# hiroyasuakada/EgoRear

Measured on AMD Instinct MI355X. Metric: 4-view frames/sec (heatmap+MVFEx+3D lift), higher is better.
Workload: dtype f32 (fp16x2 split, 22-bit operands, fp32 accumulate)

## Files before the change

egorear_amd/csrc/egr_stem_x6.hip:

```cpp
#include "egr_common.h"
#include "egr_stem_pool.h"

namespace {

typedef __bf16 bf16x8 __attribute__((ext_vector_type(8)));
typedef _Float16 f16x8 __attribute__((ext_vector_type(8)));
typedef unsigned u32x4 __attribute__((ext_vector_type(4)));

constexpr int NW = 8, NT = NW * 64;
constexpr int TH = 2 * NW, TW = 32;
constexpr int PH = 2 * TH + 5;
constexpr int PW = 2 * TW + 5;
constexpr int PWS = 72;
constexpr int PATCH = 3 * PH * PWS;
constexpr int PLOADS = (PATCH + NT - 1) / NT;
constexpr int PPAIRS = (PATCH / 2 + NT - 1) / NT;
static_assert(PATCH % 2 == 0 && PWS % 2 == 0, "pixel pairs");
#ifndef STEM_PRESPLIT
#define STEM_PRESPLIT 1
#endif
#ifndef STEM_KS
#define STEM_KS 11
#endif
constexpr int KS = STEM_KS;
// ... 325 lines not shown
        __syncthreads();
        continue;
#endif
        if constexpr (POOL) {
            StemPool<NW> pool;
            pool.reduce(acc, sc, sh, half);
            if constexpr (PRE) {
                if (next < total) publish_max(buf ^ 1, pv2);
            }
            __syncthreads();
            pool.publish(s_patch[buf], wave, l31, half);
            if constexpr (PRE) {
                if (next < total) { patch_scale(buf ^ 1, psc, pinv); park2(buf ^ 1, pv2, psc); }
            } else {
                if (next < total) park(buf ^ 1, pv);
            }
            __syncthreads();
            pool.finish(s_patch[buf], wave, l31, half, y, n, oy0, ox0, a.ho >> 1, a.wo >> 1);
            amx = fmaxf(amx, pool.amx);
        } else {
#pragma unroll
            for (int i = 0; i < 2; ++i) {
                const int oy = oy0 + 2 * wave + i;
#pragma unroll
                for (int r = 0; r < 16; ++r) {
                    const int ox = ox0 + (r & 3) + 8 * (r >> 2) + 4 * half;
                    f32x2 v;
                    v[0] = acc[i][0][r] * sc[0] + sh[0];
                    v[1] = acc[i][1][r] * sc[1] + sh[1];
                    if (!raw) {
                        v[0] = v[0] > 0.f ? v[0] : 0.f;
                        v[1] = v[1] > 0.f ? v[1] : 0.f;
                    }
                    *reinterpret_cast<f32x2*>(&y[(((int64_t)n * a.ho + oy) * a.wo + ox) * 64 + 2 * l31]) = v;
                }
            }
            if constexpr (PRE) {
                if (next < total) publish_max(buf ^ 1, pv2);
                __syncthreads();
                if (next < total) { patch_scale(buf ^ 1, psc, pinv); park2(buf ^ 1, pv2, psc); }
            } else {
                if (next < total) park(buf ^ 1, pv);
            }
            __syncthreads();
        }
    }
    if (POOL && a.amax_out) {
        amx = wave_max(amx);
        if (lane == 0 && amx > 0.f)
            __hip_atomic_fetch_max(a.amax_out + ((blockIdx.x * NW + wave) & 63), __float_as_uint(amx), __ATOMIC_RELAXED, __HIP_MEMORY_SCOPE_AGENT);
    }
}

__global__ __launch_bounds__(64) void pack_stem_w6_kernel(const float* __restrict__ w, uint8_t* __restrict__ img) {
    const int lane = threadIdx.x, j = blockIdx.x & 1, s = blockIdx.x >> 1, grp = blockIdx.y;
    const int co = 2 * (lane & 31) + j, p = 2 * s + (lane >> 5);
    const float* wr = w + ((int64_t)grp * 64 + co) * 148;
    u32x4 h, m, l;
#pragma unroll
    for (int e = 0; e < 4; ++e) {
        float v[2];
#pragma unroll
        for (int z = 0; z < 2; ++z) {
            const int kw = 2 * e + z;
            v[z] = (p <= 20 && kw < 7) ? wr[p * 7 + kw] : 0.f;
        }
        h[e] = cvt_pk_bf16(v[0], v[1]);
        const float r0 = v[0] - bf16_lo_f32(h[e]), r1 = v[1] - bf16_hi_f32(h[e]);
        m[e] = cvt_pk_bf16(r0, r1);
        l[e] = cvt_pk_bf16(r0 - bf16_lo_f32(m[e]), r1 - bf16_hi_f32(m[e]));
    }
    uint8_t* dst = img + (int64_t)grp * WBYTES + ((s * 2 + j) * 3) * 1024 + lane * 16;
    *reinterpret_cast<u32x4*>(dst) = h;
    *reinterpret_cast<u32x4*>(dst + 1024) = m;
    *reinterpret_cast<u32x4*>(dst + 2048) = l;
}

__global__ __launch_bounds__(64) void pack_stem_wh2_kernel(const float* __restrict__ w, uint8_t* __restrict__ img, float* __restrict__ descale) {
    const int lane = threadIdx.x, j = blockIdx.x & 1, s = blockIdx.x >> 1, grp = blockIdx.y;
    const int co = 2 * (lane & 31) + j, p = 2 * s + (lane >> 5);
    const float* wr = w + ((int64_t)grp * 64 + co) * 148;
    float m = 0.f;
    for (int k = 0; k < 147; ++k) m = fmaxf(m, fabsf(wr[k]));
    float sc, inv;
    pow2_prescale(__float_as_uint(m), sc, inv);
    if (s == 0 && lane < 32) descale[grp * 64 + co] = inv;
    u32x4 h, l;
#pragma unroll
    for (int e = 0; e < 4; ++e) {
        float v[2];
#pragma unroll
        for (int z = 0; z < 2; ++z) {
            const int kw = 2 * e + z;
            v[z] = (p <= 20 && kw < 7) ? wr[p * 7 + kw] : 0.f;
        }
        unsigned hh, ll;
        split2_f16(v[0], v[1], sc, hh, ll);
        h[e] = hh;
        l[e] = ll;
    }
    uint8_t* dst = img + (int64_t)grp * WBYTES2 + ((s * 2 + j) * 2) * 1024 + lane * 16;
    *reinterpret_cast<u32x4*>(dst) = h;
    *reinterpret_cast<u32x4*>(dst + 1024) = l;
}

}

extern "C" int64_t egr_stem_wh2_bytes(void) { return WBYTES2; }

extern "C" int egr_pack_stem_wh2_f32(const float* w, int32_t groups, void* img, float* descale, void* stream) {
    if (!w || !img || !descale) return EGR_ENULL;
    if (groups <= 0 || groups > 65535 || ((uintptr_t)img & 15)) return EGR_EINVAL;
    hipLaunchKernelGGL(pack_stem_wh2_kernel, dim3(KS * 2, (unsigned)groups), dim3(64), 0, (hipStream_t)stream, w, (uint8_t*)img, descale);
    return egr_launch_status();
}

extern "C" int64_t egr_stem_w6_bytes(void) { return WBYTES; }

extern "C" int egr_pack_stem_w6_f32(const float* w, int32_t groups, void* img, void* stream) {
    if (!w || !img) return EGR_ENULL;
    if (groups <= 0 || groups > 65535 || ((uintptr_t)img & 15)) return EGR_EINVAL;
    hipLaunchKernelGGL(pack_stem_w6_kernel, dim3(KS * 2, (unsigned)groups), dim3(64), 0, (hipStream_t)stream, w, (uint8_t*)img);
    return egr_launch_status();
}

static int stem_x6_run(const float* x, egr_nmap xmap, int32_t n, int32_t h, int32_t w, const void* w6, const float* scale, const float* shift,
                       float* y, int32_t pool, int32_t groups, int64_t gx, uint32_t* amax_out, void* stream, const float* wds = nullptr);

extern "C" int egr_stem_conv7x7_h2_f32(const float* x, egr_nmap xmap, int32_t n, int32_t h, int32_t w, const void* wh2, const float* w_descale,
                                       const float* scale, const float* shift, float* y, int32_t pool, int32_t groups, int64_t gx,
                                       uint32_t* amax_out, void* stream) {
    if (!w_descale) return EGR_ENULL;
    if (amax_out && !pool) return EGR_EINVAL;
    return stem_x6_run(x, xmap, n, h, w, wh2, scale, shift, y, pool, groups, gx, amax_out, stream, w_descale);
}

extern "C" int egr_stem_conv7x7_x6_f32(const float* x, egr_nmap xmap, int32_t n, int32_t h, int32_t w, const void* w6,
                                       const float* scale, const float* shift, float* y, int32_t pool, int32_t groups, int64_t gx,
                                       void* stream) {
    return stem_x6_run(x, xmap, n, h, w, w6, scale, shift, y, pool, groups, gx, nullptr, stream);
}

extern "C" int egr_stem_conv7x7_x6_ex_f32(const float* x, egr_nmap xmap, int32_t n, int32_t h, int32_t w, const void* w6,
                                          const float* scale, const float* shift, float* y, int32_t pool, int32_t groups, int64_t gx,
                                          uint32_t* amax_out, void* stream) {
    if (amax_out && !pool) return EGR_EINVAL;
    return stem_x6_run(x, xmap, n, h, w, w6, scale, shift, y, pool, groups, gx, amax_out, stream);
}

static int stem_x6_run(const float* x, egr_nmap xmap, int32_t n, int32_t h, int32_t w, const void* w6, const float* scale, const float* shift,
                       float* y, int32_t pool, int32_t groups, int64_t gx, uint32_t* amax_out, void* stream, const float* wds) {
    if (!x || !w6 || !y || ((scale == nullptr) != (shift == nullptr))) return EGR_ENULL;
    if (pool && !scale) return EGR_EINVAL;
    if (groups <= 0 || groups > 65535 || ((uintptr_t)w6 & 15)) return EGR_EINVAL;
    if (n <= 0 || h <= 0 || w <= 0 || h % (2 * TH) != 0 || w % (2 * TW) != 0 || xmap.n_inner <= 0) return EGR_EINVAL;
    StemX6Args a;
    a.x = x; a.xmap = xmap; a.n = n; a.h = h; a.w = w; a.ho = h / 2; a.wo = w / 2;
    a.w6 = (const uint8_t*)w6; a.scale = scale; a.shift = shift; a.y = y;
    a.tiles_x = a.wo / TW; a.tiles_y = a.ho / TH;
    a.gx = gx;
    a.amax_out = amax_out;
    a.wds = wds;
    const int64_t tiles = (int64_t)n * a.tiles_x * a.tiles_y;
    if (tiles >= (1LL << 31)) return EGR_EINVAL;
    int64_t blocks = 256 / groups;
    if (blocks < 1) blocks = 1;
    if (blocks > tiles) blocks = tiles;
    hipStream_t s = (hipStream_t)stream;
    if (pool) {
        stem_pool_init<NW>(y, (int64_t)groups * n, a.ho / 2, a.wo / 2, s);
        if (wds) hipLaunchKernelGGL((stem_x6_kernel<true, 2>), dim3((unsigned)blocks, (unsigned)groups), dim3(NT), 0, s, a);
        else hipLaunchKernelGGL((stem_x6_kernel<true, 3>), dim3((unsigned)blocks, (unsigned)groups), dim3(NT), 0, s, a);
    } else {
        if (wds) hipLaunchKernelGGL((stem_x6_kernel<false, 2>), dim3((unsigned)blocks, (unsigned)groups), dim3(NT), 0, s, a);
        else hipLaunchKernelGGL((stem_x6_kernel<false, 3>), dim3((unsigned)blocks, (unsigned)groups), dim3(NT), 0, s, a);
    }
    return egr_launch_status();
}
```

egorear_amd/hip.py:

```python
from __future__ import annotations

import ctypes as C
import math
import os
import threading
from typing import Optional, Union

import torch

_HERE = os.path.dirname(os.path.abspath(__file__))
LIB_PATH = os.environ.get("EGR_LIB") or os.path.join(_HERE, "csrc", "libegorear_hip.so")

ACT_NONE, ACT_RELU, ACT_GELU = 0, 1, 2
RES_NONE, RES_BEFORE_ACT, RES_AFTER_ACT, RES_UP2_BEFORE_ACT = 0, 1, 2, 3



import contextlib
import dataclasses
import sys
import types


class _on_default:
# ... 58 lines not shown
        return self.replace(w_format="f16", h2=True, layer_h2=True)

    @_on_default
    def fast_training(self) -> "LaunchPolicy":
        return self.fast().replace(train_one_product=True)

    @property
    def fp16_scheme(self) -> bool:
        return self.w_format in ("f16x2", "f16")


POLICY = LaunchPolicy.from_env()
_POLICY_TLS = threading.local()


def policy() -> LaunchPolicy:
    cur = getattr(_POLICY_TLS, "cur", None)
    return cur if cur is not None else POLICY


@contextlib.contextmanager
def use_policy(p: Optional[LaunchPolicy]):
    if p is None:
        yield
        return
    old = getattr(_POLICY_TLS, "cur", None)
    _POLICY_TLS.cur = p
    try:
        yield
    finally:
        _POLICY_TLS.cur = old


def install_policy_properties(module_name: str, mapping: dict) -> None:
    def make(field):
        return property(lambda self: getattr(policy(), field), lambda self, v: setattr(POLICY, field, v))
    mod = sys.modules[module_name]
    mod.__class__ = type("_PolicyModule", (types.ModuleType,), {name: make(field) for name, field in mapping.items()})


install_policy_properties(__name__, {
    "H2": "h2", "X6_MIN_ROWS": "x6_min_rows", "X6_MIN_FLOPS": "x6_min_flops", "X6_TRAIN_MIN_ROWS": "x6_train_min_rows",
    "X6_TRAIN_MIN_FLOPS": "x6_train_min_flops", "CHAIN": "chain", "CHAIN_MIN_ROWS": "chain_min_rows", "CHAIN_BIG": "chain_big",
    "CHAIN_BIG_MIN_ROWS": "chain_big_min_rows", "WGRAD_X6": "wgrad_x6", "WGRAD_FORCE": "wgrad_force"})

EXPORTS = [
    "egr_conv2d_nhwc_f32", "egr_stem_conv7x7_f32", "egr_maxpool_nhwc_f32", "egr_upsample2x_nhwc_f32",
    "egr_avgpool_nhwc_f32", "egr_argmax_rows_f32", "egr_layernorm_f32", "egr_joint_mha_f32", "egr_msda_gather_f32",
    "egr_fisheye_project_f32", "egr_linear_smallk_f32", "egr_jqa_sum_f32", "egr_tokens_to_nhwc_f32", "egr_version",
    "egr_device_arch", "egr_conv_force_config", "egr_preprocess_u8_f32", "egr_pose_metrics_f32", "egr_gt_heatmap_f32", "egr_conv_debug_stamps", "egr_conv2d_wgrad_f32", "egr_conv2d_masked_f32", "egr_up2_relu_head_f32",
    "egr_msda_fwd_f32", "egr_msda_bwd_f32", "egr_w6_elems", "egr_pack_w6_f32", "egr_pack_w6_many_f32", "egr_joint_layer_f32",
    "egr_preprocess_fused_u8_f32", "egr_preprocess_band_rows", "egr_preprocess_last_kernel", "egr_conv_set_persist", "egr_stem_conv7x7_pool_f32",
    "egr_stem_w6_bytes", "egr_pack_stem_w6_f32", "egr_stem_conv7x7_x6_f32", "egr_wgrad_last_kernel", "egr_conv_last_kernel", "egr_conv_set_tap", "egr_conv_set_tapx", "egr_conv_set_splitk_fused", "egr_fisheye_project2_f32", "egr_pack_layer_w_f32", "egr_pack_layer_wh2_f32",
    "egr_conv2d_nhwc_ex_f32", "egr_wh2_elems", "egr_pack_wh2_f32", "egr_absmax_f32", "egr_stem_conv7x7_x6_ex_f32", "egr_stem_wh2_bytes", "egr_pack_stem_wh2_f32", "egr_stem_conv7x7_h2_f32",
    "egr_pack_wh2_many_f32", "egr_conv2d_masked_ex_f32", "egr_conv2d_wgrad_ex_f32", "egr_wgrad_last_h2", "egr_wgrad_last_planes",
    "egr_wstream_image_bytes", "egr_pack_wstream_f32", "egr_linear_wstream_workspace_bytes", "egr_linear_wstream_f32", "egr_conv1x1_chain_f32",
    "egr_jqa_query_f32", "egr_pose_query_f32", "egr_layer_set_planes", "egr_head_set_persist", "egr_heatmap_metrics_f32",
    "egr_conv_plan", "egr_soft_argmax_f32", "egr_soft_argmax_bwd_f32", "egr_coord_l1_f32",
    "egr_triangulate_f32", "egr_triangulate_bwd_f32", "egr_volume_fuse_f32", "egr_volume_fuse_bwd_f32",
    "egr_peaks_f32", "egr_consensus_f32", "egr_skeleton_fit_f32", "egr_bone_lengths_f32", "egr_skeleton_resize_f32",
    "egr_trajectory_smooth_f32", "egr_trajectory_smooth_bwd_f32", "egr_rig_refine_f32", "egr_rig_refine_workspace_bytes",
    "egr_ray_track_f32", "egr_ray_track_workspace_bytes",
]


class NMap(C.Structure):
    _fields_ = [("n_inner", C.c_int32), ("stride_inner", C.c_int64), ("stride_outer", C.c_int64)]


class ConvDesc(C.Structure):
    _fields_ = [
        ("n", C.c_int32), ("h", C.c_int32), ("w", C.c_int32), ("cin", C.c_int32), ("cout", C.c_int32),
        ("kh", C.c_int32), ("kw", C.c_int32), ("stride", C.c_int32), ("pad", C.c_int32),
        ("ho", C.c_int32), ("wo", C.c_int32), ("ldx", C.c_int32), ("ldy", C.c_int32), ("ldr", C.c_int32),
        ("xmap", NMap), ("ymap", NMap), ("rmap", NMap),
        ("act", C.c_int32), ("res_mode", C.c_int32), ("out_nchw", C.c_int32), ("split_k", C.c_int32),
        ("groups", C.c_int32),
        ("gx", C.c_int64), ("gw", C.c_int64), ("gp", C.c_int64), ("gy", C.c_int64), ("gr", C.c_int64),
        ("grs", C.c_int64), ("grm", C.c_int64),
        ("transposed", C.c_int32), ("w_format", C.c_int32),
    ]


class ConvAux(C.Structure):
    _fields_ = [("w_descale", C.c_void_p), ("amax_in", C.c_void_p), ("amax_out", C.c_void_p),
                ("bn_partials", C.c_void_p), ("bn_tiles_out", C.c_void_p), ("bn_capacity", C.c_int64),
                ("in_mode", C.c_int32), ("in_up2_out", C.c_void_p)]


IN_PLAIN, IN_UP2_RELU = 0, 1


class ConvPlan(C.Structure):
    _fields_ = [(n, C.c_int32) for n in ("route", "bm", "bn", "variant", "planes", "tiles_m", "tiles_n", "grid_x", "grid_y", "grid_z", "block",
                                         "split_k", "ktiles_per_split", "persistent", "cls_mode", "fused_reduce", "reduce_pass", "bn_slabs")]


ROUTE_F32_TILED, ROUTE_SPLIT_TILED, ROUTE_TAP, ROUTE_TAP2, ROUTE_STREAM_1X1, ROUTE_SMALL_F32, ROUTE_TAPX = range(7)
PRE_ROUTE_LDS, PRE_ROUTE_DWORD, PRE_ROUTE_GENERIC, PRE_ROUTE_FUSED = range(4)
W_F16X2, W_F16X1, W_F16X1T = 4, 8, 16


class ChainAux(C.Structure):
    _fields_ = [("w2", C.c_void_p), ("w2_descale", C.c_void_p), ("shift1", C.c_void_p), ("cmid", C.c_int32), ("act1", C.c_int32),
                ("gw2", C.c_int64), ("gp1", C.c_int64)]


# ... 7 lines not shown
                                           "x_out", "w_ol", "b_ol", "ol_out")] +
                [("ol_n", C.c_int32), ("w_packed", C.c_int32)] +
                [(n, C.c_void_p) for n in ("lnp_g", "lnp_b", "xn_out", "w_r0", "b_r0", "w_r2", "b_r2", "anchors3d", "pred_out",
                                           "w_h0", "b_h0", "h0_out", "amax_h0")] +
                [("h0_n", C.c_int32)])


class JqaQueryDesc(C.Structure):
    _fields_ = ([(n, C.c_int32) for n in ("B", "J", "C", "groups", "kb", "pool_hw", "ol_n", "w_packed")] +
                [(n, C.c_void_p) for n in ("t", "s32", "w_hp2", "b_hp2", "w_bfb", "b_bfb", "embed", "w_q", "b_q", "w_ol", "b_ol",
                                           "x_out", "ol_out")])


class PoseQueryDesc(C.Structure):
    _fields_ = ([(n, C.c_int32) for n in ("B", "J", "C", "ol_n", "w_packed")] +
                [(n, C.c_void_p) for n in ("h1", "w_m2", "b_m2", "ctm", "cams", "w_qg0", "b_qg0", "w_qg2", "b_qg2", "w_qg4", "b_qg4",
                                           "w_ol", "b_ol", "pred_out", "anchors3d_out", "anchors2d_out", "valid_out", "x_out", "ol_out")])


def _load() -> C.CDLL:
    if not os.path.exists(LIB_PATH):
        raise ImportError(
            f"{LIB_PATH} not found: build it with `python -m egorear_amd.csrc.build` "
            "(or __graft_entry__.build()).  egorear_amd has no CPU / PyTorch fallback.")
    lib = C.CDLL(LIB_PATH)
    vp, i32, i64, f32 = C.c_void_p, C.c_int32, C.c_int64, C.c_float
    lib.egr_conv2d_nhwc_f32.argtypes = [C.POINTER(ConvDesc), vp, vp, vp, vp, vp, vp, vp, vp, vp, C.c_size_t, vp]
    lib.egr_conv2d_nhwc_ex_f32.argtypes = [C.POINTER(ConvDesc), vp, vp, vp, vp, vp, vp, vp, vp, vp, C.c_size_t, C.POINTER(ConvAux), vp]
    lib.egr_conv_plan.argtypes = [C.POINTER(ConvDesc), vp, vp, vp, vp, vp, vp, vp, vp, vp, vp, C.c_size_t, C.POINTER(ConvAux), C.POINTER(ConvPlan)]
    lib.egr_conv1x1_chain_f32.argtypes = [C.POINTER(ConvDesc), vp, vp, vp, vp, vp, C.POINTER(ConvAux), C.POINTER(ChainAux), vp]
    lib.egr_fill_f32.argtypes = [vp, f32, i64, vp]
    lib.egr_fill_f32.restype = C.c_int
    lib.egr_absmax_f32.argtypes = [vp, i64, vp, vp]
    lib.egr_wh2_elems.restype = C.c_int64
    lib.egr_wh2_elems.argtypes = [i32, i32]
    lib.egr_pack_wh2_f32.argtypes = [vp, i32, i32, i32, vp, vp, vp]
    lib.egr_stem_conv7x7_f32.argtypes = [vp, NMap, i32, i32, i32, vp, vp, vp, vp, i32, i64, vp]
    lib.egr_stem_conv7x7_pool_f32.argtypes = [vp, NMap, i32, i32, i32, vp, vp, vp, vp, i32, i64, vp]
    lib.egr_wgrad_last_kernel.argtypes = []
    lib.egr_wgrad_last_planes.argtypes = []
    lib.egr_conv_last_kernel.argtypes = []
    lib.egr_conv_set_tap.argtypes = [i32]
    lib.egr_conv_set_tapx.argtypes = [i32, i32, i32]
    lib.egr_conv_set_splitk_fused.argtypes = [i32]
    lib.egr_stem_w6_bytes.restype = C.c_int64
    lib.egr_stem_w6_bytes.argtypes = []
    lib.egr_pack_stem_w6_f32.argtypes = [vp, i32, vp, vp]
    lib.egr_stem_conv7x7_x6_f32.argtypes = [vp, NMap, i32, i32, i32, vp, vp, vp, vp, i32, i32, i64, vp]
    lib.egr_stem_conv7x7_x6_ex_f32.argtypes = [vp, NMap, i32, i32, i32, vp, vp, vp, vp, i32, i32, i64, vp, vp]
    lib.egr_stem_wh2_bytes.restype = C.c_int64
    lib.egr_stem_wh2_bytes.argtypes = []
    lib.egr_pack_stem_wh2_f32.argtypes = [vp, i32, vp, vp, vp]
    lib.egr_stem_conv7x7_h2_f32.argtypes = [vp, NMap, i32, i32, i32, vp, vp, vp, vp, vp, i32, i32, i64, vp, vp]
    lib.egr_wstream_image_bytes.restype = C.c_int64
    lib.egr_wstream_image_bytes.argtypes = [i32, i32]
    lib.egr_pack_wstream_f32.argtypes = [vp, i32, i32, vp, vp, vp]
    lib.egr_linear_wstream_workspace_bytes.restype = C.c_int64
    lib.egr_linear_wstream_workspace_bytes.argtypes = [i32, i32, i32]
    lib.egr_linear_wstream_f32.argtypes = [vp, i64, i32, i32, vp, vp, vp, i32, i32, vp, vp, i64, vp, vp, i64, vp]
    lib.egr_maxpool_nhwc_f32.argtypes = [vp, vp, i32, i32, i32, i32, i32, i32, i32, vp]
    lib.egr_upsample2x_nhwc_f32.argtypes = [vp, i32, vp, i32, i32, i32, i32, i32, i32, vp]
    lib.egr_avgpool_nhwc_f32.argtypes = [vp, vp, i32, i32, i32, vp]
    lib.egr_argmax_rows_f32.argtypes = [vp, i32, i32, i32, f32, vp, vp, vp, vp, vp]
    lib.egr_soft_argmax_f32.argtypes = [vp, i32, i32, i32, f32, i32, i32, f32, vp, vp, vp, vp, vp, vp, vp]
    lib.egr_soft_argmax_bwd_f32.argtypes = [vp, vp, vp, vp, vp, vp, i32, i32, i32, f32, i32, i32, i32, vp, vp]
    lib.egr_triangulate_f32.argtypes = [vp, vp, vp, vp, i32, i32, i32, f32, f32, f32, f32, vp, vp, vp, vp, vp]
    lib.egr_triangulate_bwd_f32.argtypes = [vp, vp, vp, vp, i32, i32, i32, f32, f32, f32, f32, vp, vp, vp, vp, vp]
    lib.egr_volume_fuse_f32.argtypes = [vp, vp, vp, vp, vp, vp, i32, i32, i32, i32, i32, i32, f32, f32, f32, vp, vp, vp, vp, vp, vp]
    lib.egr_volume_fuse_bwd_f32.argtypes = [vp, vp, vp, vp, vp, vp, i32, i32, i32, i32, i32, i32, f32, f32, f32, vp, vp, vp, vp]
    lib.egr_peaks_f32.argtypes = [vp, i32, i32, i32, i32, i32, i32, f32, f32, vp, vp, vp, vp, vp]
    lib.egr_consensus_f32.argtypes = [vp, vp, vp, vp, vp, i32, i32, i32, i32, f32, f32, f32, i32, f32, vp, vp, vp, vp, vp, vp, vp]
    lib.egr_skeleton_fit_f32.argtypes = [vp, vp, vp, vp, vp, vp, i32, vp, vp, i32, i32, i32, f32, f32, f32, f32, f32, f32, i32, vp, vp, vp, vp,
                                         vp, vp, vp, vp, vp]
    lib.egr_bone_lengths_f32.argtypes = [vp, vp, vp, i32, i32, vp, vp, vp, vp]
    lib.egr_skeleton_resize_f32.argtypes = [vp, vp, vp, vp, i32, i32, i32, vp, vp]
    lib.egr_trajectory_smooth_f32.argtypes = [vp, vp, vp, i32, i32, i32, f32, f32, f32, i32, i32, vp, vp, vp, vp, vp, vp, vp]
    lib.egr_trajectory_smooth_bwd_f32.argtypes = [vp, vp, vp, vp, i32, i32, i32, f32, f32, vp, vp, vp, vp]
    lib.egr_rig_refine_workspace_bytes.restype = C.c_int64
    lib.egr_rig_refine_workspace_bytes.argtypes = [i32, i32, i32]
    lib.egr_rig_refine_f32.argtypes = [vp, vp, vp, vp, i32, i32, i32, i32, f32, f32, f32, f32, i32, f32, i32, vp, i64, vp, vp, vp, vp, vp, vp,
                                       vp, vp, vp, vp]
    lib.egr_ray_track_workspace_bytes.restype = C.c_int64
    lib.egr_ray_track_workspace_bytes.argtypes = [i32, i32, i32, i32]
    lib.egr_ray_track_f32.argtypes = [vp, vp, vp, vp, i32, i32, i32, i32, f32, f32, f32, f32, f32, f32, i32, i32, C.c_double, vp, i64, vp, vp, vp,
                                      vp, vp, vp, vp]
    lib.egr_coord_l1_f32.argtypes = [vp, vp, vp, i32, i32, f32, vp, vp, vp]
    lib.egr_layernorm_f32.argtypes = [vp, vp, vp, vp, vp, i32, i32, f32, i32, vp]
    lib.egr_joint_mha_f32.argtypes = [vp, vp, i32, i32, i32, i32, f32, vp]
    lib.egr_msda_gather_f32.argtypes = [vp, i32, vp, i32, vp, vp, vp, i32, i32, i32, i32, i32, i32, vp, vp, vp, vp, i32, vp]
    lib.egr_fisheye_project_f32.argtypes = [vp, vp, vp, i32, i32, vp, vp, vp, vp]
    lib.egr_fisheye_project2_f32.argtypes = [vp, vp, vp, vp, i32, i32, vp, vp, vp, vp]
    lib.egr_linear_smallk_f32.argtypes = [vp, i64, i64, vp, vp, vp, i32, i32, i32, i32, i32, vp]
    lib.egr_jqa_sum_f32.argtypes = [vp, vp, vp, vp, i32, i32, i32, i32, vp]
    lib.egr_tokens_to_nhwc_f32.argtypes = [vp, vp, i32, i32, i32, vp]
    lib.egr_version.restype = C.c_char_p
    lib.egr_w6_elems.restype = C.c_int64
    lib.egr_device_arch.argtypes = [C.c_char_p, i32]
    lib.egr_conv_force_config.argtypes = [i32]
    lib.egr_conv_set_persist.argtypes = [i32, i32]
    lib.egr_up2_relu_head_f32.argtypes = [vp, i32, i32, i32, i32, vp, vp, i32, vp, i32, i64, i64, i32, i64, vp]
    lib.egr_conv2d_masked_f32.argtypes = [C.POINTER(ConvDesc), vp, vp, vp, vp, vp, vp, C.c_size_t, vp]
    lib.egr_conv2d_masked_ex_f32.argtypes = [C.POINTER(ConvDesc), vp, vp, vp, vp, vp, vp, C.c_size_t, C.POINTER(ConvAux), vp]
    lib.egr_conv2d_wgrad_f32.argtypes = [C.POINTER(ConvDesc), vp, vp, vp, vp, vp, C.c_size_t, i32, vp]
    lib.egr_conv2d_wgrad_ex_f32.argtypes = [C.POINTER(ConvDesc), vp, vp, vp, vp, vp, C.c_size_t, i32, vp, vp, vp]
    lib.egr_gt_heatmap_f32.argtypes = [vp, i32, C.c_double, i32, i32, vp, vp, vp]
    lib.egr_pose_metrics_f32.argtypes = [vp, vp, i32, i32, f32, i32, vp, vp, vp]
# ... 665 lines not shown
def pack_stem_w6(wpack: torch.Tensor) -> torch.Tensor:
    if wpack.dim() != 3 or wpack.shape[1:] != (64, 148) or wpack.dtype != torch.float32:
        raise RuntimeError("egorear_amd.pack_stem_w6: (groups, 64, 148) fp32 expected")
    img = torch.empty((wpack.shape[0], int(lib.egr_stem_w6_bytes())), device=wpack.device, dtype=torch.uint8)
    _launch("egr_pack_stem_w6_f32", lib.egr_pack_stem_w6_f32, _p(_cont(wpack, "stem weight")), wpack.shape[0], _p(img, torch.uint8), _stream())
    return img


def pack_wstream(w: torch.Tensor):
    if w.dim() != 2 or w.dtype != torch.float32 or w.shape[0] % 64 or w.shape[1] % 256:
        raise RuntimeError("egorear_amd.pack_wstream: (n % 64 == 0, k % 256 == 0) fp32 expected")
    n, k = w.shape
    img = torch.empty((int(lib.egr_wstream_image_bytes(n, k)),), device=w.device, dtype=torch.uint8)
    ds = torch.empty((n,), device=w.device, dtype=torch.float32)
    _launch("egr_pack_wstream_f32", lib.egr_pack_wstream_f32, _p(_cont(w, "weight")), n, k, _p(img, torch.uint8), _p(ds), _stream())
    return img, ds


def linear_wstream(x: torch.Tensor, img: torch.Tensor, descale: torch.Tensor, bias: Optional[torch.Tensor], act: int, workspace: torch.Tensor,
                   amax_out: Optional[torch.Tensor] = None) -> torch.Tensor:
    rec = getattr(x, "_egr_amax", None)
    if rec is None:
        raise RuntimeError("egorear_amd.linear_wstream: the rows carry no abs-max record")
    n = descale.numel()
    rows, k = x.shape
    if x.dtype != torch.float32 or x.stride(1) != 1 or img.numel() != 4 * n * k:
        raise RuntimeError("egorear_amd.linear_wstream: operands do not match")
    y = torch.empty((rows, n), device=x.device, dtype=torch.float32)
    for r0 in range(0, rows, 64):
        r = min(64, rows - r0)
        need = int(lib.egr_linear_wstream_workspace_bytes(r, n, k))
        if need < 0 or workspace.numel() * workspace.element_size() < need:
            raise RuntimeError(f"egorear_amd.linear_wstream: workspace of {need} bytes needed")
        xr, yr = x[r0:r0 + r], y[r0:r0 + r]
        _launch("egr_linear_wstream_f32", lib.egr_linear_wstream_f32, _p(xr), xr.stride(0), r, k, _p(img, torch.uint8), _p(descale),
                _p(bias), n, act, _p(rec, torch.int32), _p(yr), yr.stride(0), _p(amax_out, torch.int32), _p(workspace, workspace.dtype),
                workspace.numel() * workspace.element_size(), _stream(), flops=2.0 * r * n * k, nbytes=4.0 * n * k + 4.0 * r * (n + k),
                tag="h2 wstream")
    if amax_out is not None:
        y._egr_amax = amax_out
    return y


def pack_stem_wh2(wpack: torch.Tensor):
    if wpack.dim() != 3 or wpack.shape[1:] != (64, 148) or wpack.dtype != torch.float32:
        raise RuntimeError("egorear_amd.pack_stem_wh2: (groups, 64, 148) fp32 expected")
    img = torch.empty((wpack.shape[0], int(lib.egr_stem_wh2_bytes())), device=wpack.device, dtype=torch.uint8)
    ds = torch.empty((wpack.shape[0], 64), device=wpack.device, dtype=torch.float32)
    _launch("egr_pack_stem_wh2_f32", lib.egr_pack_stem_wh2_f32, _p(_cont(wpack, "stem weight")), wpack.shape[0], _p(img, torch.uint8), _p(ds), _stream())
    return img, ds


def stem_x6(img: torch.Tensor, view0: int, nviews: int, w6: torch.Tensor, scale, shift, groups: int = 1, pool: bool = False,
            amax_out: Optional[torch.Tensor] = None, w_descale: Optional[torch.Tensor] = None) -> Img:
    B, V, Cc, H, W = img.shape
    if Cc != 3:
        raise RuntimeError("egorear_amd.stem_x6: 3-channel input expected")
    _cont(img, "input image batch")
    raw = scale is None and shift is None
    if pool and raw:
        raise RuntimeError("egorear_amd.stem_x6: the fused max-pool needs the eval-mode BatchNorm scale / shift")
    h2 = w_descale is not None
    if (view0 + groups * nviews > V or w6.dtype != torch.uint8
            or w6.numel() != groups * int(lib.egr_stem_wh2_bytes() if h2 else lib.egr_stem_w6_bytes())
            or (h2 and w_descale.numel() != groups * 64)
            or (not raw and (scale.numel() != groups * 64 or shift.numel() != groups * 64))):
        raise RuntimeError("egorear_amd.stem_x6: views / weights mismatch")
    n = nviews * B
    d = 4 if pool else 2
    y = torch.empty((groups * n, H // d, W // d, 64), device=img.device, dtype=torch.float32)
    base = img.reshape(-1)[view0 * 3 * H * W:]
    xmap = NMap(B, V * 3 * H * W, 3 * H * W)
    if amax_out is not None and (not pool or amax_out.numel() != 64 or amax_out.dtype != torch.int32):
        raise RuntimeError("egorear_amd.stem_x6: the abs-max record (64 int32 slots) goes with pool=True")
    if h2:
        _launch("egr_stem_conv7x7_x6_f32", lib.egr_stem_conv7x7_h2_f32, _p(base), xmap, n, H, W, _p(_cont(w6, "stem weight"), torch.uint8),
                _p(_cont(w_descale, "stem descale")), _p(scale), _p(shift), _p(y), 1 if pool else 0, groups, nviews * 3 * H * W,
                _p(amax_out, torch.int32), _stream(),
                flops=2.0 * groups * n * (H // 2) * (W // 2) * 64 * 147, nbytes=4.0 * groups * n * (3 * H * W + (H // d) * (W // d) * 64),
                tag="h2 pool" if pool else "h2")
    else:
        _launch("egr_stem_conv7x7_x6_f32", lib.egr_stem_conv7x7_x6_ex_f32, _p(base), xmap, n, H, W, _p(_cont(w6, "stem weight"), torch.uint8), _p(scale),
                _p(shift), _p(y), 1 if pool else 0, groups, nviews * 3 * H * W, _p(amax_out, torch.int32), _stream(),
                flops=2.0 * groups * n * (H // 2) * (W // 2) * 64 * 147, nbytes=4.0 * groups * n * (3 * H * W + (H // d) * (W // d) * 64),
                tag="x6 pool" if pool else "x6")
    out = Img(y)
    out.tag(amax_out)
    return out


def maxpool(x: Img, k: int, stride: int, pad: int) -> Img:
    if not x.t.is_contiguous():
        raise RuntimeError("egorear_amd.maxpool: contiguous NHWC input expected")
    ho = (x.h + 2 * pad - k) // stride + 1
    wo = (x.w + 2 * pad - k) // stride + 1
    y = torch.empty((x.n, ho, wo, x.c), device=x.t.device, dtype=torch.float32)
    _launch("egr_maxpool_nhwc_f32", lib.egr_maxpool_nhwc_f32, _p(x.t), _p(y), x.n, x.h, x.w, x.c, k, stride, pad, _stream(),
            nbytes=4.0 * x.n * x.c * (x.h * x.w + ho * wo))
    out = Img(y)
    out.tag(x.amax)
    return out


def upsample2x(x: Img, out: Optional[Img] = None, relu: bool = False) -> Img:
    if x.n > 1 and x.nstride != x.h * x.w * x.ld:
        raise RuntimeError("egorear_amd.upsample2x: images must be densely stacked")
    if out is None:
        out = Img(torch.empty((x.n, 2 * x.h, 2 * x.w, x.c), device=x.t.device, dtype=torch.float32))
    if (out.n, out.h, out.w, out.c) != (x.n, 2 * x.h, 2 * x.w, x.c) or (out.n > 1 and out.nstride != out.h * out.w * out.ld):
        raise RuntimeError("egorear_amd.upsample2x: bad output view")
    _launch("egr_upsample2x_nhwc_f32", lib.egr_upsample2x_nhwc_f32, _p(x.t), x.ld, _p(out.t), out.ld, x.n, x.h, x.w, x.c, 1 if relu else 0, _stream(),
            nbytes=4.0 * 5 * x.n * x.h * x.w * x.c)
    out.tag(x.amax)
    return out


def up2_relu_head(lo: Img, wgt: torch.Tensor, bias: Optional[torch.Tensor], planes: torch.Tensor, ymap: NMap, gy: int, groups: int = 1):
    if not lo.t.is_contiguous() or lo.n % groups:
        raise RuntimeError("egorear_amd.up2_relu_head: dense NHWC input with groups | n expected")
    cout, cin = wgt.shape[-2], wgt.shape[-1]
    npg = lo.n // groups
    if cin != lo.c or wgt.numel() != groups * cout * cin or (bias is not None and bias.numel() != groups * cout):
        raise RuntimeError("egorear_amd.up2_relu_head: weight / bias shape")
    ho, wo = 2 * lo.h, 2 * lo.w
    last = (groups - 1) * gy + (npg - 1) // ymap.n_inner * ymap.stride_outer + min(npg - 1, ymap.n_inner - 1) * ymap.stride_inner + cout * ho * wo
    if not planes.is_contiguous() or last > planes.numel():
        raise RuntimeError("egorear_amd.up2_relu_head: output map runs outside the tensor")
    _launch("egr_up2_relu_head_f32", lib.egr_up2_relu_head_f32, _p(lo.t), lo.n, lo.h, lo.w, cin, _p(_cont(wgt, "weight")), _p(bias), cout,
            _p(planes), ymap.n_inner, ymap.stride_inner, ymap.stride_outer, groups, gy, _stream(),
# ... 930 lines not shown
```

include/egorear_hip.h:

```cpp
#ifndef EGOREAR_HIP_H
#define EGOREAR_HIP_H

#include <stddef.h>
#include <stdint.h>

#ifdef __cplusplus
extern "C" {
#endif

#define EGR_EINVAL (-1)
#define EGR_ENULL (-2)
#define EGR_EWORKSPACE (-3)

enum { EGR_ACT_NONE = 0, EGR_ACT_RELU = 1, EGR_ACT_GELU = 2 };
enum { EGR_RES_NONE = 0, EGR_RES_BEFORE_ACT = 1, EGR_RES_AFTER_ACT = 2,
       EGR_RES_UP2_BEFORE_ACT = 3  };

typedef struct {
    int32_t n_inner;
    int64_t stride_inner;
    int64_t stride_outer;
} egr_nmap;

typedef struct {
// ... 104 lines not shown
                  const float* workspace, size_t workspace_floats, const egr_conv_aux* aux, egr_conv_plan_t* out);

int egr_conv2d_wgrad_f32(const egr_conv_desc* d, const float* x, const float* dy, float* dw, float* db,
                         float* workspace, size_t workspace_floats, int32_t accumulate, void* stream);
int egr_conv2d_wgrad_ex_f32(const egr_conv_desc* d, const float* x, const float* dy, float* dw, float* db, float* workspace,
                            size_t workspace_floats, int32_t accumulate, const uint32_t* amax_x, const uint32_t* amax_dy, void* stream);
int egr_wgrad_last_h2(void);
int egr_wgrad_last_planes(void);
int egr_wgrad_last_kernel(void);

int egr_conv_force_config(int cfg);
int egr_conv_last_kernel(void);
int egr_conv_set_splitk_fused(int on);
int egr_conv_set_tap(int on);
int egr_conv_set_tapx(int32_t on, int32_t min_tiles, int32_t blocks);
int egr_conv_set_persist(int slots, int max_ktiles);

int egr_up2_relu_head_f32(const float* lo, int32_t n, int32_t h, int32_t w, int32_t cin, const float* wgt, const float* bias,
                          int32_t cout, float* planes, int32_t n_inner, int64_t stride_inner, int64_t stride_outer,
                          int32_t groups, int64_t gy, void* stream);
int egr_head_set_persist(int on);

int egr_conv_debug_stamps(unsigned long long* buf);

int egr_stem_conv7x7_f32(const float* x, egr_nmap xmap, int32_t n, int32_t h, int32_t w,
                         const float* wpack, const float* scale, const float* shift, float* y,
                         int32_t groups ,
                         int64_t gx, void* stream);

int egr_stem_conv7x7_pool_f32(const float* x, egr_nmap xmap, int32_t n, int32_t h, int32_t w,
                              const float* wpack, const float* scale, const float* shift, float* y,
                              int32_t groups, int64_t gx, void* stream);

int64_t egr_stem_w6_bytes(void);
int egr_pack_stem_w6_f32(const float* w, int32_t groups, void* w6, void* stream);
int egr_stem_conv7x7_x6_f32(const float* x, egr_nmap xmap, int32_t n, int32_t h, int32_t w,
                            const void* w6, const float* scale, const float* shift, float* y,
                            int32_t pool, int32_t groups, int64_t gx, void* stream);
int egr_stem_conv7x7_x6_ex_f32(const float* x, egr_nmap xmap, int32_t n, int32_t h, int32_t w,
                            const void* w6, const float* scale, const float* shift, float* y,
                            int32_t pool, int32_t groups, int64_t gx, uint32_t* amax_out, void* stream);
int64_t egr_wstream_image_bytes(int32_t n, int32_t k);
int egr_pack_wstream_f32(const float* w, int32_t n, int32_t k, void* img, float* descale, void* stream);
int64_t egr_linear_wstream_workspace_bytes(int32_t rows, int32_t n, int32_t k);
int egr_linear_wstream_f32(const float* x, int64_t ldx, int32_t rows, int32_t k, const void* wimg, const float* w_descale, const float* bias,
                           int32_t n, int32_t act, const uint32_t* amax_in, float* y, int64_t ldy, uint32_t* amax_out, void* workspace,
                           int64_t workspace_bytes, void* stream);

int64_t egr_stem_wh2_bytes(void);
int egr_pack_stem_wh2_f32(const float* w, int32_t groups, void* img, float* descale, void* stream);
int egr_stem_conv7x7_h2_f32(const float* x, egr_nmap xmap, int32_t n, int32_t h, int32_t w, const void* wh2, const float* w_descale,
                            const float* scale, const float* shift, float* y, int32_t pool, int32_t groups, int64_t gx,
                            uint32_t* amax_out, void* stream);

int egr_maxpool_nhwc_f32(const float* x, float* y, int32_t n, int32_t h, int32_t w, int32_t c,
                         int32_t k, int32_t stride, int32_t pad, void* stream);

int egr_upsample2x_nhwc_f32(const float* x, int32_t ldx, float* y, int32_t ldy,
                            int32_t n, int32_t h, int32_t w, int32_t c, int32_t relu, void* stream);

int egr_absmax_f32(const float* x, int64_t n, uint32_t* record, void* stream);

int egr_avgpool_nhwc_f32(const float* x, float* y, int32_t n, int32_t hw, int32_t c, void* stream);

int egr_argmax_rows_f32(const float* hm, int32_t rows, int32_t hgt, int32_t wid, float thr,
                        float* anchors , float* maxvals, uint8_t* valid, int32_t* index, void* stream);

int egr_soft_argmax_f32(const float* hm, int32_t rows, int32_t hgt, int32_t wid, float beta, int32_t mode, int32_t normalize, float thr,
                        float* coords , float* maxvals, int32_t* index, uint8_t* valid, float* stat ,
                        float* probs , void* stream);
int egr_soft_argmax_bwd_f32(const float* hm, const float* stat, const float* coords, const int32_t* index, const float* g_coords,
                            const float* g_maxvals , int32_t rows, int32_t hgt, int32_t wid, float beta, int32_t mode,
                            int32_t normalize, int32_t accumulate, float* g_hm, void* stream);
int egr_coord_l1_f32(const float* coords, const int32_t* index, const uint8_t* valid, int32_t rows, int32_t wid, float weight,
                     double* loss, float* g_coords , void* stream);

int egr_triangulate_f32(const float* coords, const float* conf, const float* cams, const float* ctm , int32_t B, int32_t V,
                        int32_t J, float sx, float sy, float threshold, float min_det_ratio, float* pts ,
                        float* cost , float* resid , uint8_t* ok , void* stream);
int egr_triangulate_bwd_f32(const float* coords, const float* conf, const float* cams, const float* ctm , int32_t B,
                            int32_t V, int32_t J, float sx, float sy, float threshold, float min_det_ratio,
                            const float* g_pts , const float* g_cost , float* g_coords, float* g_conf,
                            void* stream);

int egr_volume_fuse_f32(const float* hm, const float* conf, const float* centers, const float* cams, const float* ctm ,
                        const uint8_t* center_ok , int32_t B, int32_t V, int32_t J, int32_t H, int32_t W, int32_t G,
                        float cube, float beta, float threshold, float* pose , float* peak ,
                        int32_t* index , float* spread , uint8_t* ok , void* stream);
int egr_volume_fuse_bwd_f32(const float* hm, const float* conf, const float* centers, const float* cams, const float* ctm ,
                            const uint8_t* center_ok , int32_t B, int32_t V, int32_t J, int32_t H, int32_t W, int32_t G,
                            float cube, float beta, float threshold, const float* g_pose ,
                            const float* g_peak , float* g_hm, void* stream);

int egr_peaks_f32(const float* hm, int32_t rows, int32_t hgt, int32_t wid, int32_t K, int32_t nms_radius, int32_t refine_radius, float beta,
                  float min_score, float* coords , float* score , int32_t* index ,
                  int32_t* count , void* stream);
int egr_consensus_f32(const float* cand, const float* cscore, const int32_t* cindex, const float* cams, const float* ctm ,
                      int32_t B, int32_t V, int32_t J, int32_t K, float sx, float sy, float max_reproj, int32_t min_views,
                      float min_det_ratio, int32_t* choice , float* sel_coords ,
                      float* sel_conf , float* score , int32_t* inliers , int32_t* hyp ,
                      void* stream);

int egr_skeleton_fit_f32(const float* coords, const float* conf, const float* cams, const float* ctm ,
                         const int32_t* parents , const float* bone_length, int32_t bone_length_per_frame, const float* init,
                         const uint8_t* init_ok, int32_t B, int32_t V, int32_t J, float sx, float sy, float threshold, float min_det_ratio,
                         float lambda, float rho, int32_t iterations, float* pose , float* ray_cost ,
// ... 147 lines not shown
```

Baseline: 6973.

## Add warp-specialized stem conv kernel splitting MFMA and load/store waves

```diff
diff --git a/egorear_amd/csrc/egr_stem_x6.hip b/egorear_amd/csrc/egr_stem_x6.hip
--- a/egorear_amd/csrc/egr_stem_x6.hip
+++ b/egorear_amd/csrc/egr_stem_x6.hip
@@ -401,6 +401,292 @@
     }
 }
 
+namespace rs {
+constexpr int MW = 4;
+constexpr int LT = MW * 64;
+constexpr int LPAIRS = (PATCH / 2 + LT - 1) / LT;
+constexpr int ROWF = 16 * 64;
+constexpr int O_MAIN = 0;
+constexpr int O_NEXT = O_MAIN + 8 * ROWF * 4;
+constexpr int O_EA = O_NEXT + MW * ROWF * 4;
+constexpr int O_EB = O_EA + 8 * 64 * 4;
+constexpr int O_PMAX = O_EB + MW * 64 * 4;
+constexpr int O_PATCH = O_PMAX + 4 * MW * 4;
+constexpr int PBYTES = PATCH * 4;
+constexpr int O_W = O_PATCH + 2 * PBYTES;
+constexpr int LDS_BYTES = O_W + WBYTES2;
+static_assert(O_PATCH % 16 == 0 && O_W % 16 == 0 && LDS_BYTES <= 160 * 1024, "LDS map");
+}
+
+__global__ __launch_bounds__(NT, 1) void stem_h2_pool_rs_kernel(const StemX6Args a) {
+    using namespace rs;
+    __shared__ __attribute__((aligned(16))) uint8_t lds[LDS_BYTES];
+    const int tid = threadIdx.x, lane = tid & 63, wave = __builtin_amdgcn_readfirstlane(tid >> 6);
+    const int grp = blockIdx.y;
+    const int tpi = a.tiles_x * a.tiles_y;
+    const int total = a.n * tpi;
+    const int ntiles = (total - (int)blockIdx.x + (int)gridDim.x - 1) / (int)gridDim.x;
+    const int pho = a.ho >> 1, pwo = a.wo >> 1;
+    const auto barrier = [] { asm volatile("s_waitcnt lgkmcnt(0)\n\ts_barrier" ::: "memory"); };
+    unsigned* const s_pmax = reinterpret_cast<unsigned*>(lds + O_PMAX);
+    auto patch_scale = [&](int slot, float& s, float& inv) {
+        unsigned m = s_pmax[slot * MW + (lane & (MW - 1))];
+#pragma unroll
+        for (int o = MW / 2; o > 0; o >>= 1) {
+            const unsigned other = (unsigned)__shfl_xor((int)m, o, 64);
+            m = other > m ? other : m;
+        }
+        pow2_prescale(__builtin_amdgcn_readfirstlane(m), s, inv);
+    };
+    {
+        const u32x4* src = reinterpret_cast<const u32x4*>(a.w6 + (int64_t)grp * WBYTES2);
+        for (int i = tid; i < WBYTES2 / 16; i += NT) reinterpret_cast<u32x4*>(lds + O_W)[i] = src[i];
+    }
+
+    if (wave < MW) {
+        const int l31 = lane & 31, half = lane >> 5;
+        float sc[2], sh[2], wds[2];
+#pragma unroll
+        for (int j = 0; j < 2; ++j) {
+            sc[j] = a.scale[grp * 64 + 2 * l31 + j];
+            sh[j] = a.shift[grp * 64 + 2 * l31 + j];
+            wds[j] = a.wds[grp * 64 + 2 * l31 + j];
+        }
+        const int abase = ((2 * (4 * wave)) * PWS + 2 * l31) >> 1;
+        unsigned bbase = O_W + lane * 16;
+        asm volatile("" : "+v"(bbase));
+        float amx = 0.f;
+        barrier();
+        barrier();
+        for (int it = 0; it < ntiles; ++it) {
+            const unsigned* const ph = reinterpret_cast<const unsigned*>(lds + O_PATCH + (it & 1) * PBYTES);
+            float psc, pinv;
+            patch_scale(it & 3, psc, pinv);
+            f32x16 acc[2][2][2];
+#pragma unroll
+            for (int p = 0; p < 2; ++p)
+#pragma unroll
+                for (int i = 0; i < 2; ++i)
+#pragma unroll
+                    for (int j = 0; j < 2; ++j)
+#pragma unroll
+                        for (int r = 0; r < 16; ++r) acc[p][i][j][r] = 0.f;
+            u32x4 al[4], ah[2][4];
+            u32x4 bl[2], bh[2][2];
+            auto read_a = [&](int s, int pl, u32x4 (&d)[4]) {
+                const unsigned* const q = ph + abase + pl * (PATCH / 2) + ((half ? pair_off_t<PH>(2 * s + 1) : pair_off_t<PH>(2 * s)) >> 1);
+#pragma unroll
+                for (int i = 0; i < 4; ++i)
+#pragma unroll
+                    for (int e = 0; e < 4; ++e) d[i][e] = q[i * PWS + e];
+            };
+            auto read_b = [&](int s, int pl, u32x4 (&d)[2]) {
+#pragma unroll
+                for (int j = 0; j < 2; ++j) d[j] = *reinterpret_cast<const u32x4*>(lds + bbase + ((s * 2 + j) * 2 + pl) * 1024);
+            };
+            auto mul = [&](const u32x4 (&fa)[4], const u32x4 (&fb)[2]) {
+#pragma unroll
+                for (int i = 0; i < 4; ++i)
+#pragma unroll
+                    for (int j = 0; j < 2; ++j)
+                        acc[i >> 1][i & 1][j] = __builtin_amdgcn_mfma_f32_32x32x16_f16(__builtin_bit_cast(f16x8, fa[i]), __builtin_bit_cast(f16x8, fb[j]),
+                                                                                      acc[i >> 1][i & 1][j], 0, 0, 0);
+            };
+            read_a(0, 1, al);
+            read_b(0, 0, bh[0]);
+            read_a(0, 0, ah[0]);
+            read_b(0, 1, bl);
+#pragma unroll
+            for (int s = 0; s < KS; ++s) {
+                const int par = s & 1;
+                if (s + 1 < KS) {
+                    read_b(s + 1, 0, bh[par ^ 1]);
+                    read_a(s + 1, 0, ah[par ^ 1]);
+                }
+                __builtin_amdgcn_sched_barrier(0);
+                mul(al, bh[par]);
+                __builtin_amdgcn_sched_barrier(0);
+                if (s + 1 < KS) read_a(s + 1, 1, al);
+                __builtin_amdgcn_sched_barrier(0);
+                mul(ah[par], bl);
+                __builtin_amdgcn_sched_barrier(0);
+                if (s + 1 < KS) read_b(s + 1, 1, bl);
+                __builtin_amdgcn_sched_barrier(0);
+                mul(ah[par], bh[par]);
+                __builtin_amdgcn_sched_barrier(0);
+            }
+#pragma unroll
+            for (int p = 0; p < 2; ++p)
+#pragma unroll
+                for (int i = 0; i < 2; ++i)
+#pragma unroll
+                    for (int j = 0; j < 2; ++j) {
+                        const float dsc = pinv * wds[j];
+#pragma unroll
+                        for (int r = 0; r < 16; ++r) acc[p][i][j][r] *= dsc;
+                    }
+            StemPool<NW> pa, pb;
+            pa.reduce(acc[0], sc, sh, half);
+            pb.reduce(acc[1], sc, sh, half);
+            amx = fmaxf(amx, fmaxf(pa.amx, pb.amx));
+            barrier();
+            float* const st = reinterpret_cast<float*>(lds);
+#pragma unroll
+            for (int q = 0; q < 8; ++q) {
+                const int o = StemPool<NW>::pc(q, half) * 64 + 2 * l31;
+                f32x2 mid;
+                mid[0] = fmaxf(pb.P0[q][0], pa.P1[q][0]);
+                mid[1] = fmaxf(pb.P0[q][1], pa.P1[q][1]);
+                *reinterpret_cast<f32x2*>(&st[O_MAIN / 4 + (2 * wave) * ROWF + o]) = pa.P0[q];
+                *reinterpret_cast<f32x2*>(&st[O_MAIN / 4 + (2 * wave + 1) * ROWF + o]) = mid;
+                *reinterpret_cast<f32x2*>(&st[O_NEXT / 4 + wave * ROWF + o]) = pb.P1[q];
+            }
+            if (half) {
+                f32x2 mid;
+                mid[0] = fmaxf(pb.e0[0], pa.e1[0]);
+                mid[1] = fmaxf(pb.e0[1], pa.e1[1]);
+                *reinterpret_cast<f32x2*>(&st[O_EA / 4 + (2 * wave) * 64 + 2 * l31]) = pa.e0;
+                *reinterpret_cast<f32x2*>(&st[O_EA / 4 + (2 * wave + 1) * 64 + 2 * l31]) = mid;
+                *reinterpret_cast<f32x2*>(&st[O_EB / 4 + wave * 64 + 2 * l31]) = pb.e1;
+            }
+            barrier();
+        }
+        if (a.amax_out) {
+            amx = wave_max(amx);
+            if (lane == 0 && amx > 0.f)
+                __hip_atomic_fetch_max(a.amax_out + ((blockIdx.x * NW + wave) & 63), __float_as_uint(amx), __ATOMIC_RELAXED, __HIP_MEMORY_SCOPE_AGENT);
+        }
+    } else {
+        const int lw = wave - MW, ltid = tid - LT;
+        const float* const xg = a.x + grp * a.gx;
+        float* const y = a.y + (int64_t)grp * a.n * pho * pwo * 64;
+        int q_geo[LPAIRS], q_off[LPAIRS];
+#pragma unroll
+        for (int u = 0; u < LPAIRS; ++u) {
+            const int i = 2 * (ltid + LT * u);
+            const int ci = i / (PH * PWS);
+            const int r = i - ci * PH * PWS;
+            const int py = r / PWS, px = r - py * PWS;
+            q_geo[u] = (i < PATCH) ? ((py << 8) | px) : (1 << 30);
+            q_off[u] = (ci * a.h + py) * a.w + px;
+        }
+        auto tile_of = [&](int it) { return (int)blockIdx.x + it * (int)gridDim.x; };
+        auto fetch = [&](int tile, float (&v)[2 * LPAIRS]) {
+            const int n = tile / tpi;
+            const int t = tile - n * tpi;
+            const int ty = t / a.tiles_x, tx = t - ty * a.tiles_x;
+            const int iy0 = 2 * ty * TH - 3, ix0 = 2 * tx * TW - 3;
+            const uint64_t ip = (uint64_t)(xg + egr_map(a.xmap, n));
+            const uint32_t ip_lo = __builtin_amdgcn_readfirstlane((uint32_t)ip), ip_hi = __builtin_amdgcn_readfirstlane((uint32_t)(ip >> 32));
+            const __amdgpu_buffer_rsrc_t rx = __builtin_amdgcn_make_buffer_rsrc((void*)(((uint64_t)ip_hi << 32) | ip_lo), 0, 0x80000000u, 0x00020000);
+            const int toff = iy0 * a.w + ix0;
+            const unsigned xlim = (unsigned)(a.w < ix0 + PW ? a.w : ix0 + PW);
+#pragma unroll
+            for (int u = 0; u < LPAIRS; ++u) {
+                const int g = q_geo[u];
+                const int iy = iy0 + (g >> 8), ix = ix0 + (g & 255);
+                const bool rowok = (unsigned)iy < (unsigned)a.h;
+                const int o = (int)((unsigned)(toff + q_off[u]) * 4u);
+                const int o0 = (rowok && (unsigned)ix < xlim) ? o : (int)0x80000000;
+                const int o1 = (rowok && (unsigned)(ix + 1) < xlim) ? o + 4 : (int)0x80000000;
+                v[2 * u] = __builtin_bit_cast(float, __builtin_amdgcn_raw_buffer_load_b32(rx, o0, 0, 0));
+                v[2 * u + 1] = __builtin_bit_cast(float, __builtin_amdgcn_raw_buffer_load_b32(rx, o1, 0, 0));
+            }
+        };
+        auto publish_max = [&](int slot, const float (&v)[2 * LPAIRS]) {
+            float m = 0.f;
+#pragma unroll
+            for (int u = 0; u < 2 * LPAIRS; ++u) m = fmaxf(m, fabsf(v[u]));
+            m = wave_max(m);
+            if (lane == 0) s_pmax[slot * MW + lw] = __float_as_uint(m);
+        };
+        auto park = [&](int buf, const float (&v)[2 * LPAIRS], float psc) {
+            unsigned pbase = O_PATCH + buf * PBYTES + ltid * 4;
+            asm volatile("" : "+v"(pbase));
+            unsigned* const ph = reinterpret_cast<unsigned*>(lds + pbase);
+#pragma unroll
+            for (int u = 0; u < LPAIRS; ++u)
+                if (LT * (u + 1) <= PATCH / 2 || ltid + LT * u < PATCH / 2) {
+                    unsigned h, l;
+                    split2_f16(v[2 * u], v[2 * u + 1], psc, h, l);
+                    ph[LT * u] = h;
+                    ph[PATCH / 2 + LT * u] = l;
+                }
+        };
+        auto amax4 = [](float* p, f32x4 v) {
+#pragma unroll
+            for (int c = 0; c < 4; ++c) atomicMax(reinterpret_cast<int*>(p) + c, __float_as_int(v[c]));
+        };
+        auto max4 = [](f32x4 x, f32x4 z) {
+            f32x4 r;
+#pragma unroll
+            for (int c = 0; c < 4; ++c) r[c] = fmaxf(x[c], z[c]);
+            return r;
+        };
+        auto finish = [&](int tile) {
+            const float* const st = reinterpret_cast<const float*>(lds);
+            const int n = tile / tpi;
+            const int t = tile - n * tpi;
+            const int ty = t / a.tiles_x, tx = t - ty * a.tiles_x;
+            const int gp0 = ty * (TH / 2), gc0 = tx * (TW / 2);
+            const bool top = ty > 0, left = tx > 0, right = gc0 + 16 < pwo, bottom = gp0 + TH / 2 < pho;
+#pragma unroll
+            for (int rr = 0; rr < 2; ++rr) {
+                const int row = 2 * lw + rr;
+                float* const yrow = y + (((int64_t)n * pho + gp0 + row) * pwo + gc0) * 64;
+                const bool joined = rr == 0 && lw > 0;
+#pragma unroll
+                for (int k = 0; k < 4; ++k) {
+                    const int o = k * 256 + lane * 4;
+                    f32x4 v = *reinterpret_cast<const f32x4*>(&st[O_MAIN / 4 + row * ROWF + o]);
+                    if (joined) v = max4(v, *reinterpret_cast<const f32x4*>(&st[O_NEXT / 4 + (lw - 1) * ROWF + o]));
+                    if ((row == 0 && top) || (k == 0 && lane < 16 && left)) amax4(yrow + o, v);
+                    else *reinterpret_cast<f32x4*>(yrow + o) = v;
+                }
+                if (right) {
+                    float e = st[O_EA / 4 + row * 64 + lane];
+                    if (joined) e = fmaxf(e, st[O_EB / 4 + (lw - 1) * 64 + lane]);
+                    atomicMax(reinterpret_cast<int*>(yrow + ROWF + lane), __float_as_int(e));
+                }
+            }
+            if (lw == MW - 1 && bottom) {
+                float* const yrow = y + (((int64_t)n * pho + gp0 + TH / 2) * pwo + gc0) * 64;
+#pragma unroll
+                for (int k = 0; k < 4; ++k) {
+                    const int o = k * 256 + lane * 4;
+                    amax4(yrow + o, *reinterpret_cast<const f32x4*>(&st[O_NEXT / 4 + (MW - 1) * ROWF + o]));
+                }
+                if (right) atomicMax(reinterpret_cast<int*>(yrow + ROWF + lane), __float_as_int(st[O_EB / 4 + (MW - 1) * 64 + lane]));
+            }
+        };
+
+        float pv[2 * LPAIRS];
+        float psc, pinv;
+        fetch(tile_of(0), pv);
+        publish_max(0, pv);
+        barrier();
+        patch_scale(0, psc, pinv);
+        park(0, pv, psc);
+        if (ntiles > 1) {
+            fetch(tile_of(1), pv);
+            publish_max(1, pv);
+        }
+        barrier();
+        for (int it = 0; it < ntiles; ++it) {
+            if (it + 1 < ntiles) {
+                patch_scale((it + 1) & 3, psc, pinv);
+                park((it + 1) & 1, pv, psc);
+            }
+            if (it + 2 < ntiles) fetch(tile_of(it + 2), pv);
+            if (it > 0) finish(tile_of(it - 1));
+            if (it + 2 < ntiles) publish_max((it + 2) & 3, pv);
+            barrier();
+            barrier();
+        }
+        finish(tile_of(ntiles - 1));
+    }
+}
+
 __global__ __launch_bounds__(64) void pack_stem_w6_kernel(const float* __restrict__ w, uint8_t* __restrict__ img) {
     const int lane = threadIdx.x, j = blockIdx.x & 1, s = blockIdx.x >> 1, grp = blockIdx.y;
     const int co = 2 * (lane & 31) + j, p = 2 * s + (lane >> 5);
@@ -474,7 +760,8 @@
 }
 
 static int stem_x6_run(const float* x, egr_nmap xmap, int32_t n, int32_t h, int32_t w, const void* w6, const float* scale, const float* shift,
-                       float* y, int32_t pool, int32_t groups, int64_t gx, uint32_t* amax_out, void* stream, const float* wds = nullptr);
+                       float* y, int32_t pool, int32_t groups, int64_t gx, uint32_t* amax_out, void* stream, const float* wds = nullptr,
+                       bool role_split = true);
 
 extern "C" int egr_stem_conv7x7_h2_f32(const float* x, egr_nmap xmap, int32_t n, int32_t h, int32_t w, const void* wh2, const float* w_descale,
                                        const float* scale, const float* shift, float* y, int32_t pool, int32_t groups, int64_t gx,
@@ -484,6 +771,14 @@
     return stem_x6_run(x, xmap, n, h, w, wh2, scale, shift, y, pool, groups, gx, amax_out, stream, w_descale);
 }
 
+extern "C" int egr_stem_conv7x7_h2_ref_f32(const float* x, egr_nmap xmap, int32_t n, int32_t h, int32_t w, const void* wh2, const float* w_descale,
+                                           const float* scale, const float* shift, float* y, int32_t pool, int32_t groups, int64_t gx,
+                                           uint32_t* amax_out, void* stream) {
+    if (!w_descale) return EGR_ENULL;
+    if (amax_out && !pool) return EGR_EINVAL;
+    return stem_x6_run(x, xmap, n, h, w, wh2, scale, shift, y, pool, groups, gx, amax_out, stream, w_descale, false);
+}
+
 extern "C" int egr_stem_conv7x7_x6_f32(const float* x, egr_nmap xmap, int32_t n, int32_t h, int32_t w, const void* w6,
                                        const float* scale, const float* shift, float* y, int32_t pool, int32_t groups, int64_t gx,
                                        void* stream) {
@@ -498,7 +793,8 @@
 }
 
 static int stem_x6_run(const float* x, egr_nmap xmap, int32_t n, int32_t h, int32_t w, const void* w6, const float* scale, const float* shift,
-                       float* y, int32_t pool, int32_t groups, int64_t gx, uint32_t* amax_out, void* stream, const float* wds) {
+                       float* y, int32_t pool, int32_t groups, int64_t gx, uint32_t* amax_out, void* stream, const float* wds, bool role_split) {
+    static const int g_role_split = getenv("EGR_STEM_ROLE_SPLIT") ? atoi(getenv("EGR_STEM_ROLE_SPLIT")) != 0 : 1;
     if (!x || !w6 || !y || ((scale == nullptr) != (shift == nullptr))) return EGR_ENULL;
     if (pool && !scale) return EGR_EINVAL;
     if (groups <= 0 || groups > 65535 || ((uintptr_t)w6 & 15)) return EGR_EINVAL;
@@ -518,7 +814,9 @@
     hipStream_t s = (hipStream_t)stream;
     if (pool) {
         stem_pool_init<NW>(y, (int64_t)groups * n, a.ho / 2, a.wo / 2, s);
-        if (wds) hipLaunchKernelGGL((stem_x6_kernel<true, 2>), dim3((unsigned)blocks, (unsigned)groups), dim3(NT), 0, s, a);
+        if (wds && role_split && g_role_split && 12LL * h * w < (1LL << 31))
+            hipLaunchKernelGGL(stem_h2_pool_rs_kernel, dim3((unsigned)blocks, (unsigned)groups), dim3(NT), 0, s, a);
+        else if (wds) hipLaunchKernelGGL((stem_x6_kernel<true, 2>), dim3((unsigned)blocks, (unsigned)groups), dim3(NT), 0, s, a);
         else hipLaunchKernelGGL((stem_x6_kernel<true, 3>), dim3((unsigned)blocks, (unsigned)groups), dim3(NT), 0, s, a);
     } else {
         if (wds) hipLaunchKernelGGL((stem_x6_kernel<false, 2>), dim3((unsigned)blocks, (unsigned)groups), dim3(NT), 0, s, a);
diff --git a/egorear_amd/hip.py b/egorear_amd/hip.py
--- a/egorear_amd/hip.py
+++ b/egorear_amd/hip.py
@@ -134,7 +134,7 @@
     "egr_msda_fwd_f32", "egr_msda_bwd_f32", "egr_w6_elems", "egr_pack_w6_f32", "egr_pack_w6_many_f32", "egr_joint_layer_f32",
     "egr_preprocess_fused_u8_f32", "egr_preprocess_band_rows", "egr_preprocess_last_kernel", "egr_conv_set_persist", "egr_stem_conv7x7_pool_f32",
     "egr_stem_w6_bytes", "egr_pack_stem_w6_f32", "egr_stem_conv7x7_x6_f32", "egr_wgrad_last_kernel", "egr_conv_last_kernel", "egr_conv_set_tap", "egr_conv_set_tapx", "egr_conv_set_splitk_fused", "egr_fisheye_project2_f32", "egr_pack_layer_w_f32", "egr_pack_layer_wh2_f32",
-    "egr_conv2d_nhwc_ex_f32", "egr_wh2_elems", "egr_pack_wh2_f32", "egr_absmax_f32", "egr_stem_conv7x7_x6_ex_f32", "egr_stem_wh2_bytes", "egr_pack_stem_wh2_f32", "egr_stem_conv7x7_h2_f32",
+    "egr_conv2d_nhwc_ex_f32", "egr_wh2_elems", "egr_pack_wh2_f32", "egr_absmax_f32", "egr_stem_conv7x7_x6_ex_f32", "egr_stem_wh2_bytes", "egr_pack_stem_wh2_f32", "egr_stem_conv7x7_h2_f32", "egr_stem_conv7x7_h2_ref_f32",
     "egr_pack_wh2_many_f32", "egr_conv2d_masked_ex_f32", "egr_conv2d_wgrad_ex_f32", "egr_wgrad_last_h2", "egr_wgrad_last_planes",
     "egr_wstream_image_bytes", "egr_pack_wstream_f32", "egr_linear_wstream_workspace_bytes", "egr_linear_wstream_f32", "egr_conv1x1_chain_f32",
     "egr_jqa_query_f32", "egr_pose_query_f32", "egr_layer_set_planes", "egr_head_set_persist", "egr_heatmap_metrics_f32",
@@ -248,6 +248,7 @@
     lib.egr_stem_wh2_bytes.argtypes = []
     lib.egr_pack_stem_wh2_f32.argtypes = [vp, i32, vp, vp, vp]
     lib.egr_stem_conv7x7_h2_f32.argtypes = [vp, NMap, i32, i32, i32, vp, vp, vp, vp, vp, i32, i32, i64, vp, vp]
+    lib.egr_stem_conv7x7_h2_ref_f32.argtypes = lib.egr_stem_conv7x7_h2_f32.argtypes
     lib.egr_wstream_image_bytes.restype = C.c_int64
     lib.egr_wstream_image_bytes.argtypes = [i32, i32]
     lib.egr_pack_wstream_f32.argtypes = [vp, i32, i32, vp, vp, vp]
@@ -1019,7 +1020,7 @@
 
 
 def stem_x6(img: torch.Tensor, view0: int, nviews: int, w6: torch.Tensor, scale, shift, groups: int = 1, pool: bool = False,
-            amax_out: Optional[torch.Tensor] = None, w_descale: Optional[torch.Tensor] = None) -> Img:
+            amax_out: Optional[torch.Tensor] = None, w_descale: Optional[torch.Tensor] = None, role_split: bool = True) -> Img:
     B, V, Cc, H, W = img.shape
     if Cc != 3:
         raise RuntimeError("egorear_amd.stem_x6: 3-channel input expected")
@@ -1041,7 +1042,7 @@
     if amax_out is not None and (not pool or amax_out.numel() != 64 or amax_out.dtype != torch.int32):
         raise RuntimeError("egorear_amd.stem_x6: the abs-max record (64 int32 slots) goes with pool=True")
     if h2:
-        _launch("egr_stem_conv7x7_x6_f32", lib.egr_stem_conv7x7_h2_f32, _p(base), xmap, n, H, W, _p(_cont(w6, "stem weight"), torch.uint8),
+        _launch("egr_stem_conv7x7_x6_f32", lib.egr_stem_conv7x7_h2_f32 if role_split else lib.egr_stem_conv7x7_h2_ref_f32, _p(base), xmap, n, H, W, _p(_cont(w6, "stem weight"), torch.uint8),
                 _p(_cont(w_descale, "stem descale")), _p(scale), _p(shift), _p(y), 1 if pool else 0, groups, nviews * 3 * H * W,
                 _p(amax_out, torch.int32), _stream(),
                 flops=2.0 * groups * n * (H // 2) * (W // 2) * 64 * 147, nbytes=4.0 * groups * n * (3 * H * W + (H // d) * (W // d) * 64),
diff --git a/include/egorear_hip.h b/include/egorear_hip.h
--- a/include/egorear_hip.h
+++ b/include/egorear_hip.h
@@ -180,6 +180,9 @@
 int egr_stem_conv7x7_h2_f32(const float* x, egr_nmap xmap, int32_t n, int32_t h, int32_t w, const void* wh2, const float* w_descale,
                             const float* scale, const float* shift, float* y, int32_t pool, int32_t groups, int64_t gx,
                             uint32_t* amax_out, void* stream);
+int egr_stem_conv7x7_h2_ref_f32(const float* x, egr_nmap xmap, int32_t n, int32_t h, int32_t w, const void* wh2, const float* w_descale,
+                                const float* scale, const float* shift, float* y, int32_t pool, int32_t groups, int64_t gx,
+                                uint32_t* amax_out, void* stream);
 
 int egr_maxpool_nhwc_f32(const float* x, float* y, int32_t n, int32_t h, int32_t w, int32_t c,
                          int32_t k, int32_t stride, int32_t pad, void* stream);
```

New measurement: 7010, median of 6. No clear change (+0.5%).
